# fakufaku/diffusion-separation

Hardware: AMD Instinct MI355X
Metric: separated utterances/sec (4 s, 8 kHz, 2-spk, N=30 PC steps) (higher is better)
Workload: dtype f16; 1 GPU; configs[1]: 2-spk N=30 PC sampler (+1 ald2 corrector step), batch=16 x 4.0 s @ 8 kHz per GPU and step, NCSN++ nf=64 random-init, 60 NFE/step; 4 consecutive steps (batches) in flight per GPU; batch_per_gpu=16, samples=32000, N=30, corrector_steps=1, nf=64, graph=True, batches_in_flight=4

## Files before the change

### diffusion-separation_amd/csrc/conv3x3_rw.hip

```cpp
#include <stdlib.h>

#ifdef RW_TIMING
#define HALO_TIMING rw
#endif
#include "conv3x3_halo.h"

namespace {

constexpr int KC = 64;
constexpr int NKB = KC / 16;
constexpr int KSC = 9 * NKB;
static_assert(KC * 2 + 16 == AROW && KC / 8 == PPL, "a pixel's chunk is one 128-byte line");

struct RwK {
  const bf16_t* x; long x_bs; int ldx; int C1;
  const bf16_t* x2; long x2_bs; int ldx2;
  const bf16_t* w; int w_chunked;
  const bf16_t* wfrag; const bf16_t* swfrag;
  const float* gn_scale; const float* gn_shift;
  const long long* gn_acc1; const long long* gn_acc2; const float* gn_gamma; const float* gn_beta;
  int gn_groups; float gn_inv_count; float gn_eps;
  const float* bias; const float* bias_b; int bias_b_ld;
  const bf16_t* res; long res_bs; int ldr;
  float out_scale;
  bf16_t* y; long y_bs; int ldy;
  long long* stats;
  const bf16_t* sx; long sx_bs; int ldsx; int sC1;
  const bf16_t* sx2; long sx2_bs; int ldsx2;
  const bf16_t* sw; int sw_chunked; int sw_shift; int sCin;
  int H, W, G, tiles_x, tiles_per_img;
  int dbg;
};

#ifndef RW_NWL2
#define RW_NWL2 8
#endif
constexpr int rw_lds_ksteps(int nch, int rpw, int nsk, int ncg) { return ncg == 4 ? nch * KSC - 64 + nsk * NKB : (nch == 2 ? RW_NWL2 : 0); }

template <int NCH, int RPW, int NSK, int NCG>
struct RwGeom {
  static constexpr int CO = 32 * NCG, PGN = 4 / NCG;
  static constexpr int TH = PGN * RPW, HH_ = TH + 2, HP = HH_ * HW_;
  static constexpr int NI = TH * TW * PPL / NT, NBP = HP - TH * TW, NB = (NBP * PPL + NT - 1) / NT;
  static constexpr int NL = NI + NB;
  static_assert(NT / PPL == TW && TH * TW * PPL % NT == 0, "one staging pass = one tile row");
  static constexpr int LDS_A = NL * (NT / PPL) * AROW;
  static constexpr int CIN = NCH * KC, SCIN = NSK * KC;
  static constexpr int LDS_TAB = (2 * CIN + CO) * 4;
  static constexpr int LDS_DESC = NB * NT * 4;
  static_assert((NI + NB) * (NT / PPL) >= HP + NB * (NT / PPL) - NBP, "dummy pixels of the last border pass fit the slot");
  static constexpr int NPH = NCH + NSK;
  static constexpr int NKS = NCH * KSC + NSK * NKB;
  static constexpr int NWL = rw_lds_ksteps(NCH, RPW, NSK, NCG), NWR = NKS - NWL;
  static constexpr int LDS_WL = NWL * NCG * 64 * 16;
  static constexpr int WL_STEP = NCG * 64 * 16;
  static constexpr int OFF_TAB = 2 * LDS_A, OFF_WL = OFF_TAB + ((LDS_TAB + 15) & ~15), OFF_DESC = OFF_WL + LDS_WL;
  static constexpr int LDS_TOTAL = OFF_DESC + LDS_DESC;
  static constexpr int chunk_of(int P) { return P < NSK ? NCH + P : P - NSK; }
  static_assert(LDS_TOTAL <= 160 * 1024, "LDS budget of one CU");
  static_assert(NT * 36 * 4 <= LDS_TOTAL, "the statistics reduce reuses the block's LDS");
};

template <int NCH, int RPW, int NSK, int MODE, int NCG>
__global__ __launch_bounds__(NT, 1) void conv3x3_rw_kernel(RwK p) {
  using G = RwGeom<NCH, RPW, NSK, NCG>;
  constexpr int CO = G::CO, PGN = G::PGN;
  constexpr int TH = G::TH, HP = G::HP, LDS_A = G::LDS_A, NL = G::NL, NPH = G::NPH, NKS = G::NKS, CIN = G::CIN, NWR = G::NWR;
  extern __shared__ __attribute__((aligned(16))) char smem[];
  char* sA = smem;
  float* sTab = reinterpret_cast<float*>(smem + G::OFF_TAB);
  int* sDesc = reinterpret_cast<int*>(smem + G::OFF_DESC);
  const int tid = threadIdx.x;
  const int lane = tid & 63, wave = __builtin_amdgcn_readfirstlane(tid >> 6);
  const int l32 = lane & 31, h = lane >> 5;
  const int cg = wave % NCG, pg = wave / NCG;
  const int b = blockIdx.x / p.G, part = blockIdx.x % p.G;
  const int t0 = (int)((long)part * p.tiles_per_img / p.G);
  const int nt = (int)((long)(part + 1) * p.tiles_per_img / p.G) - t0;
  RT_DECL

  static_assert(CIN <= NT && CO <= NT, "one table entry per thread");
  constexpr int CPG_MAX = 8;
  long long t_s[CPG_MAX], t_q[CPG_MAX];
  float t_gam = 1.f, t_bet = 0.f, t_sc = 1.f, t_sh = 0.f, t_bias = 0.f;
#pragma unroll
  for (int j = 0; j < CPG_MAX; ++j) { t_s[j] = 0; t_q[j] = 0; }
  if (tid < CIN) {
    const int c = tid;
    if (p.gn_acc1) {
      const int C1 = p.C1, C2 = CIN - C1;
      const int cpg = CIN / p.gn_groups, g0 = (c / cpg) * cpg;
#pragma unroll
      for (int j = 0; j < CPG_MAX; ++j) {
        if (j < cpg) {
          const int cc = g0 + j;
          const long long* src = cc < C1 ? p.gn_acc1 + ((long)b * C1 + cc) * 2 : p.gn_acc2 + ((long)b * C2 + (cc - C1)) * 2;
          t_s[j] = src[0];
          t_q[j] = src[1];
        }
      }
      t_gam = p.gn_gamma ? p.gn_gamma[c] : 1.f;
      t_bet = p.gn_beta ? p.gn_beta[c] : 0.f;
    } else if (p.gn_scale) {
      t_sc = p.gn_scale[(long)b * CIN + c];
      t_sh = p.gn_shift[(long)b * CIN + c];
    }
  }
  if (tid < CO) t_bias = (p.bias ? p.bias[tid] : 0.f) + (p.bias_b ? p.bias_b[(long)b * p.bias_b_ld + tid] : 0.f);
  auto build_tables = [&]() __attribute__((always_inline)) {
    if (tid < CIN) {
      float sc = t_sc, sh = t_sh;
      if (p.gn_acc1) {
        long long t_ssum = 0, t_ssq = 0;
#pragma unroll
        for (int j = 0; j < CPG_MAX; ++j) { t_ssum += t_s[j]; t_ssq += t_q[j]; }
        ds_gn_affine_from_acc(t_ssum, t_ssq, p.gn_inv_count, p.gn_eps, t_gam, t_bet, sc, sh);
      }
      sTab[tid] = sc;
      sTab[CIN + tid] = sh;
    }
    if (tid < CO) sTab[2 * CIN + tid] = t_bias * p.out_scale;
  };
  const int slot = tid & (PPL - 1);
  constexpr int NI = G::NI, NB = G::NB, NBP = G::NBP;
  const int ixp = tid / PPL;
  unsigned fl = 0;
  int dstb[NB];
#pragma unroll
  for (int kb = 0; kb < NB; ++kb) {
    const int bi = ixp + (NT / PPL) * kb;
    int hy, hx;
    if (bi < HW_) { hy = 0; hx = bi; }
    else if (bi < 2 * HW_) { hy = G::HH_ - 1; hx = bi - HW_; }
    else if (bi < 2 * HW_ + TH) { hy = 1 + bi - 2 * HW_; hx = 0; }
    else { hy = 1 + bi - 2 * HW_ - TH; hx = HW_ - 1; }
    const bool in = bi < NBP;
    const unsigned flg = in ? (hy == 0 ? 1u : 0u) | (hy == G::HH_ - 1 ? 2u : 0u) | (hx == 0 ? 4u : 0u) | (hx == HW_ - 1 ? 8u : 0u) : 16u;
    sDesc[kb * NT + tid] = in ? (hy - 1) * p.W + (hx - 1) : 0;
    dstb[kb] = (in ? hy * HW_ + hx : HP + (bi - NBP)) * AROW + slot * 16;
    fl |= flg << (5 * kb);
  }
  const int ldi0 = (HW_ + 1 + ixp) * AROW + slot * 16;

  RT_MARK(6)
  const int M = p.H * p.W;
  const __amdgpu_buffer_rsrc_t rx1 = rsrc(p.x + (long)b * p.x_bs, (unsigned)M * p.ldx * 2u);
  const __amdgpu_buffer_rsrc_t rx2 = p.x2 ? rsrc(p.x2 + (long)b * p.x2_bs, (unsigned)M * p.ldx2 * 2u) : rx1;
  const __amdgpu_buffer_rsrc_t rs1 = NSK ? rsrc(p.sx + (long)b * p.sx_bs, (unsigned)M * p.ldsx * 2u) : rx1;
  const __amdgpu_buffer_rsrc_t rs2 = (NSK && p.sx2) ? rsrc(p.sx2 + (long)b * p.sx2_bs, (unsigned)M * p.ldsx2 * 2u) : rs1;
  const __amdgpu_buffer_rsrc_t ry = rsrc(p.y + (long)b * p.y_bs, (unsigned)M * p.ldy * 2u);

  u32x4_t wf[NWR > 0 ? NWR : 1];
  char* sWl = smem + G::OFF_WL + (cg * 64 + lane) * 16;
  auto put_w = [&](int ks, const u32x4_t& v) __attribute__((always_inline)) {
    if (ks < NWR) wf[ks] = v;
    else if (pg == 0) *reinterpret_cast<u32x4_t*>(sWl + (ks - NWR) * G::WL_STEP) = v;
  };
  auto load_weights = [&]() __attribute__((always_inline)) {
    const bool wfm = p.wfrag != nullptr, sfm = NSK && p.swfrag != nullptr;
    const __amdgpu_buffer_rsrc_t rw = rsrc(wfm ? p.wfrag : p.w, 9u * CO * CIN * 2u);
    const __amdgpu_buffer_rsrc_t rsw = (NSK && p.sw) ? rsrc(sfm ? p.swfrag : p.sw, (unsigned)CO * G::SCIN * 2u) : rsrc(p.w, 0u);
    const unsigned vfrag = (unsigned)((cg * 64 + lane) * 16);
    const int co = cg * 32 + l32;
    const bool wc = p.w_chunked != 0;
    const unsigned vlane = wfm ? vfrag : (wc ? (unsigned)((co * 32 + h * 8) * 2) : (unsigned)((co * 9 * CIN + h * 8) * 2));
    const bool sc_ = NSK && p.sw_chunked != 0;
    const int kcs = sc_ ? p.sw_chunked : 16;
    const unsigned vl2 = sfm ? vfrag : (sc_ ? (unsigned)((co * kcs + h * 8) * 2) : (unsigned)((co * G::SCIN + h * 8) * 2));
    auto load_one = [&](int ks) __attribute__((always_inline)) {
      if (ks < NCH * KSC) {
        const int c = ks / KSC, tap = (ks % KSC) / NKB, kb = ks % NKB;
        const int chb = c * KC + kb * 16;
        const unsigned so = wfm ? (unsigned)(ks * NCG * 1024)
                                : (wc ? (unsigned)((((chb >> 5) * 9 + tap) * CO * 32 + (chb & 31)) * 2) : (unsigned)((tap * CIN + chb) * 2));
        put_w(ks, ld16v(rw, vlane, so));
      } else {
        const int chb = (ks - NCH * KSC) * 16;
        const unsigned so = sfm ? (unsigned)((ks - NCH * KSC) * NCG * 1024)
                                : (sc_ ? (unsigned)((((chb >> p.sw_shift) * CO) * kcs + (chb & (kcs - 1))) * 2) : (unsigned)(chb * 2));
        u32x4_t f = ld16v(rsw, vl2, so);
        if (!p.sw) {
          const int d = co - (chb + 8 * h);
#pragma unroll
          for (int e = 0; e < 4; ++e) f[e] = d == 2 * e ? DS_H_ONE : (d == 2 * e + 1 ? DS_H_ONE << 16 : 0u);
        }
        put_w(ks, f);
      }
    };
#pragma unroll
    for (int ks = NWR; ks < NKS; ++ks) load_one(ks);
#pragma unroll
    for (int ks = 0; ks < NWR; ++ks) load_one(ks);
  };

  u32x4_t pa[NL];
  struct TileG { int pix0; unsigned edge; };
  auto geom_at = [&](int ty, int tx, bool valid) {
    TileG g;
    const int y0 = ty * TH, x0 = tx * TW;
    g.edge = (y0 == 0 ? 1u : 0u) | (y0 + TH == p.H ? 2u : 0u) | (x0 == 0 ? 4u : 0u) | (x0 + TW == p.W ? 8u : 0u);
    g.pix0 = valid ? y0 * p.W + x0 : 0x3fffff;
    return g;
  };
  auto tile_geom = [&](int i) {
    const int t = t0 + i;
    const int ty = t / p.tiles_x;
    return geom_at(ty, t - ty * p.tiles_x, i < nt);
  };
  auto piece_ok = [&](auto P_, const TileG& g, int k) __attribute__((always_inline)) {
    constexpr int P = decltype(P_)::value;
    const unsigned em = (P < NCH ? (g.edge | 16u) : 31u) << (5 * (k - NI));
    return (fl & em) == 0u;
  };
  auto issue_one = [&](auto P_, const TileG& g, int k, int rel) __attribute__((always_inline)) {
    constexpr int P = decltype(P_)::value;
    constexpr bool CONV = P < NCH;
    constexpr int CB = (CONV ? P : P - NCH) * KC;
    const int c1 = CONV ? p.C1 : p.sC1;
    const bool second = CB >= c1;
    const unsigned ld2 = (unsigned)(CONV ? (second ? p.ldx2 : p.ldx) : (second ? p.ldsx2 : p.ldsx)) * 2u;
    const unsigned co2 = (unsigned)((second ? CB - c1 : CB) * 2) + (unsigned)slot * 16u;
    const __amdgpu_buffer_rsrc_t r = CONV ? (second ? rx2 : rx1) : (second ? rs2 : rs1);
    if constexpr (!CONV) {
      if (k >= NI) return;
    }
    if (k < NI) {
      const unsigned off = __umul24((unsigned)(g.pix0 + k * p.W + ixp), ld2) + co2;
      pa[k] = ld16v(r, off, 0);
      return;
    }
    const unsigned off = __umul24((unsigned)(rel + g.pix0), ld2) + co2;
#ifdef RW_TIMING
    pa[k] = ld16v(r, (piece_ok(P_, g, k) && !(p.dbg & 2)) ? off : OOB, 0);
#else
    pa[k] = ld16v(r, piece_ok(P_, g, k) ? off : OOB, 0);
#endif
  };
  constexpr bool FOLD = MODE == 2 && NSK == 0;
#if defined(DS_HALF_F16) && !defined(RW_ACT_F32)
  constexpr bool ACT_PK = true;
#else
  constexpr bool ACT_PK = false;
#endif
  constexpr int PIPE_LAG = 2;
  float gsc[ACT_PK ? 1 : 8], gsh[ACT_PK ? 1 : 8];
  unsigned psc[ACT_PK ? 4 : 1], psh[ACT_PK ? 4 : 1];
  auto act_tab = [&](int c) __attribute__((always_inline)) {
    if constexpr (MODE != 0) {
      const float4* ts = reinterpret_cast<const float4*>(sTab + c * KC + slot * 8);
      const float4* th = reinterpret_cast<const float4*>(sTab + CIN + c * KC + slot * 8);
      const float4 s0 = ts[0], s1 = ts[1], h0 = th[0], h1 = th[1];
      float a[8] = {s0.x, s0.y, s0.z, s0.w, s1.x, s1.y, s1.z, s1.w}, b_[8] = {h0.x, h0.y, h0.z, h0.w, h1.x, h1.y, h1.z, h1.w};
      if constexpr (FOLD) {
#pragma unroll
        for (int j = 0; j < 8; ++j) { a[j] *= -1.4426950408889634f; b_[j] *= -1.4426950408889634f; }
      }
      if constexpr (ACT_PK) {
#pragma unroll
        for (int d = 0; d < 4; ++d) { psc[d] = pack_h2(a[2 * d], a[2 * d + 1]); psh[d] = pack_h2(b_[2 * d], b_[2 * d + 1]); }
      } else {
#pragma unroll
        for (int j = 0; j < 8; ++j) { gsc[j] = a[j]; gsh[j] = b_[j]; }
      }
    }
  };
  u32x4_t so;
  float uz[3][2], ut[3][2];
  unsigned uzp[3], utp[3], uxp[3], udp[3], urp[3];
  auto unit_s01 = [&](auto P1_, int u0, int u1) __attribute__((always_inline)) {
    constexpr int P1 = decltype(P1_)::value;
    if constexpr (P1 < NCH && MODE != 0) {
      const int q0 = u0 >= 0 ? u0 % 3 : 0, q1 = u1 >= 0 ? u1 % 3 : 0;
      if constexpr (ACT_PK) {
        unsigned z = 0, x = 0, e = 0, dd = 0, r = 0;
        if (u0 >= 0) {
          asm("v_pk_fma_f16 %0, %1, %2, %3" : "=v"(z) : "v"(pa[u0 >> 2][u0 & 3]), "v"(psc[u0 & 3]), "v"(psh[u0 & 3]));
          x = z;
          if constexpr (MODE == 2 && !FOLD) asm("v_pk_mul_f16 %0, %1, %2" : "=v"(x) : "v"(z), "s"(0xbdc5bdc5u));
        }
        if constexpr (MODE == 2) {
          if (u1 >= 0) asm("v_pk_add_f16 %0, %1, %2" : "=v"(dd) : "v"(utp[q1]), "s"(0x3c003c00u));
          if (u0 >= 0) asm("v_exp_f16 %0, %1" : "=v"(e) : "v"(x));
          if (u1 >= 0) asm("v_rcp_f16 %0, %1" : "=v"(r) : "v"(dd));
          if (u0 >= 0) asm("v_exp_f16_sdwa %0, %1 dst_sel:WORD_1 dst_unused:UNUSED_PRESERVE src0_sel:WORD_1" : "+v"(e) : "v"(x));
          if (u1 >= 0) asm("v_rcp_f16_sdwa %0, %1 dst_sel:WORD_1 dst_unused:UNUSED_PRESERVE src0_sel:WORD_1" : "+v"(r) : "v"(dd));
          if (u1 >= 0) urp[q1] = r;
          if (u0 >= 0) utp[q0] = e;
        }
        if (u0 >= 0) uzp[q0] = z;
      } else {
        if (u1 >= 0 && MODE == 2) {
          ut[q1][0] = __builtin_amdgcn_rcpf(1.0f + ut[q1][0]);
          ut[q1][1] = __builtin_amdgcn_rcpf(1.0f + ut[q1][1]);
        }
        if (u0 >= 0) {
          const unsigned w = pa[u0 >> 2][u0 & 3];
          const int d = u0 & 3;
          const float lo = h_lo(w), hi = h_hi(w);
          const float z0 = fmaf(lo, gsc[2 * d], gsh[2 * d]), z1 = fmaf(hi, gsc[2 * d + 1], gsh[2 * d + 1]);
          uz[q0][0] = z0; uz[q0][1] = z1;
          if (MODE == 2) {
            ut[q0][0] = __builtin_amdgcn_exp2f(FOLD ? z0 : z0 * -1.4426950408889634f);
            ut[q0][1] = __builtin_amdgcn_exp2f(FOLD ? z1 : z1 * -1.4426950408889634f);
          }
        }
      }
    }
  };
  auto unit_s2x = [&](auto P1_, auto P2_, auto FIN_, const TileG& g1, const TileG& g2, int sl, int u, int rel) __attribute__((always_inline)) {
    constexpr int P1 = decltype(P1_)::value;
    constexpr bool FIN_ONLY = decltype(FIN_)::value;
    const int k = u >> 2, d = u & 3, q = u % 3;
    if constexpr (!FIN_ONLY) {
    if constexpr (P1 < NCH && MODE != 0) {
      if constexpr (ACT_PK) {
        unsigned v = uzp[q];
        if constexpr (MODE == 2) asm volatile("v_pk_mul_f16 %0, %1, %2" : "=v"(v) : "v"(uzp[q]), "v"(urp[q]));
        so[d] = v;
      } else {
        float z0 = uz[q][0], z1 = uz[q][1];
        if (MODE == 2) { z0 *= ut[q][0]; z1 *= ut[q][1]; }
        so[d] = pack_h2(z0, z1);
      }
    } else {
      so[d] = pa[k][d];
    }
    }
    if (d == 3) {
      if (P1 < NCH && MODE != 0 && k >= NI) {
        const bool ok = piece_ok(P1_, g1, k);
        so.x = ok ? so.x : 0u;
        so.y = ok ? so.y : 0u;
        so.z = ok ? so.z : 0u;
        so.w = ok ? so.w : 0u;
      }
#ifdef RW_ABL_NOLDSW
      asm volatile("" :: "v"(so));
#else
      if (P1 < NCH || k < NI)
        *reinterpret_cast<u32x4_t*>(sA + sl * LDS_A + (k < NI ? ldi0 + k * HW_ * AROW : dstb[k < NI ? 0 : k - NI])) = so;
#endif
#ifdef RW_ABL_NOLOAD
      pa[k][0] += rel;
#else
      issue_one(P2_, g2, k, rel);
#endif
    }
  };
  auto unit_s2 = [&](auto P1_, auto P2_, const TileG& g1, const TileG& g2, int sl, int u, int rel) __attribute__((always_inline)) {
    unit_s2x(P1_, P2_, std::false_type{}, g1, g2, sl, u, rel);
  };
  auto unit_fin = [&](auto P1_, auto P2_, const TileG& g1, const TileG& g2, int sl, int u, int rel) __attribute__((always_inline)) {
    unit_s2x(P1_, P2_, std::true_type{}, g1, g2, sl, u, rel);
  };
  auto unit = [&](auto P1_, auto P2_, const TileG& g1, const TileG& g2, int sl, int u, int rel) __attribute__((always_inline)) {
    unit_s01(P1_, u, -1);
    unit_s01(P1_, -1, u);
    unit_s2(P1_, P2_, g1, g2, sl, u, rel);
  };

  f32x16 acc[RPW];
#pragma unroll
  for (int r = 0; r < RPW; ++r)
#pragma unroll
    for (int e = 0; e < 16; ++e) acc[r][e] = 0.f;
  float ssum[16], ssq[16];
#pragma unroll
  for (int j = 0; j < 16; ++j) { ssum[j] = 0.f; ssq[j] = 0.f; }
  const bool has_stats = p.stats != nullptr;
  const float osc = FOLD ? p.out_scale * -0.6931471805599453f : p.out_scale;
  const int fbase = (pg * RPW * HW_ + l32) * AROW + h * 16;

  auto swap_halves = [&](u32x4_t& v) __attribute__((always_inline)) {
    auto r0 = __builtin_amdgcn_permlane32_swap(v.x, v.z, false, false);
    auto r1 = __builtin_amdgcn_permlane32_swap(v.y, v.w, false, false);
    v.x = r0[0]; v.z = r0[1]; v.y = r1[0]; v.w = r1[1];
  };
  u32x4_t ov0;
  const int srow = lane >> 4;
  const unsigned spiece = (unsigned)(cg * 64 + (srow & 1) * 32 + (srow >> 1) * 16);
  auto epi_unit = [&](const TileG& g, int r, int j, const float4& t0, const float4& t1) __attribute__((always_inline)) {
    float v[8];
    v[0] = fmaf(acc[r][8 * j + 0], osc, t0.x); v[1] = fmaf(acc[r][8 * j + 1], osc, t0.y);
    v[2] = fmaf(acc[r][8 * j + 2], osc, t0.z); v[3] = fmaf(acc[r][8 * j + 3], osc, t0.w);
    v[4] = fmaf(acc[r][8 * j + 4], osc, t1.x); v[5] = fmaf(acc[r][8 * j + 5], osc, t1.y);
    v[6] = fmaf(acc[r][8 * j + 6], osc, t1.z); v[7] = fmaf(acc[r][8 * j + 7], osc, t1.w);
#ifndef RW_ABL_NOSTATS
#pragma unroll
    for (int e = 0; e < 8; ++e) {
      ssum[8 * j + e] += v[e];
      ssq[8 * j + e] = fmaf(v[e], v[e], ssq[8 * j + e]);
    }
#endif
    u32x4_t ov = {pack_h2(v[0], v[1]), pack_h2(v[2], v[3]), pack_h2(v[4], v[5]), pack_h2(v[6], v[7])};
    swap_halves(ov);
    if (j == 0) {
      ov0 = ov;
    } else {
      u32x4_t a = ov0, b2 = ov;
#pragma unroll
      for (int d = 0; d < 4; ++d) {
        auto q = __builtin_amdgcn_permlane16_swap(a[d], b2[d], false, false);
        a[d] = q[0]; b2[d] = q[1];
      }
      const int pix = g.pix0 + (pg * RPW + r) * p.W + (lane & 15);
      const unsigned o = __umul24((unsigned)pix, (unsigned)p.ldy * 2u) + spiece;
#ifdef RW_TIMING
      const unsigned o1 = (p.dbg & 1) ? OOB : o, o2 = (p.dbg & 1) ? OOB : o + 16u * (unsigned)p.ldy * 2u;
#else
      const unsigned o1 = o, o2 = o + 16u * (unsigned)p.ldy * 2u;
#endif
#ifdef RW_ABL_NOSTORE
      asm volatile("" :: "v"(a), "v"(b2), "v"(o1), "v"(o2));
#else
      __builtin_amdgcn_raw_buffer_store_b128(a, ry, o1, 0, 0);
      __builtin_amdgcn_raw_buffer_store_b128(b2, ry, o2, 0, 0);
#endif
    }
  };
  constexpr bool REL_REGS = NWR * 4 <= 176 || NCG == 4;
  constexpr bool BIAS_REGS = true;
  float4 breg[2][2];
  int relreg[G::NB];
  auto epi_bias = [&](int j, float4& t0, float4& t1) __attribute__((always_inline)) {
    if constexpr (BIAS_REGS) {
      t0 = breg[j][0];
      t1 = breg[j][1];
    } else {
      t0 = *reinterpret_cast<const float4*>(sTab + 2 * CIN + cg * 32 + 8 * (2 * j) + 4 * h);
      t1 = *reinterpret_cast<const float4*>(sTab + 2 * CIN + cg * 32 + 8 * (2 * j + 1) + 4 * h);
    }
  };

  constexpr int RH = RPW / 2;
#ifndef RW_W_E
#define RW_W_E 2
#define RW_W_N 5
#endif
  constexpr int W_E = RW_W_E, W_N = RW_W_N;
  float et[2][2] = {{0.f, 0.f}, {0.f, 0.f}};
  u32x4_t osa = {0, 0, 0, 0}, osb = {0, 0, 0, 0};
  auto half = [&](auto P_, auto HF_, auto EPI_, int slot_r, const TileG& ge, const TileG& g1, const TileG& g2) __attribute__((always_inline)) {
    constexpr int P = decltype(P_)::value, HF = decltype(HF_)::value;
    constexpr bool EPI = decltype(EPI_)::value;
    constexpr int C = G::chunk_of(P);
    constexpr bool CONV = C < NCH;
    constexpr int NK = CONV ? KSC : NKB;
    constexpr int W0 = CONV ? C * KSC : NCH * KSC + (C - NCH) * NKB;
    constexpr int C1 = G::chunk_of((P + 1) % NPH), C2 = G::chunk_of((P + 2) % NPH);
    constexpr int NU = NL * 4;
    constexpr bool ACT1 = C1 < NCH && MODE != 0;
    constexpr int LAG = ACT1 ? PIPE_LAG : 0, NUV = NU + LAG, NLU = 2 * NUV;
    constexpr int NGH = NK * RH;
    constexpr int w0 = (P == 0) ? W_E : W_N, w1 = (P == NPH - 1) ? W_E : W_N, CAP = NGH * (w0 + w1);
    auto lub = [](int GP) constexpr { return NLU * (GP <= NGH ? GP * w0 : NGH * w0 + (GP - NGH) * w1) / CAP; };
    constexpr int NLE = RH * 22;
    constexpr int R0 = HF * RH, ER0 = HF ? 0 : RH;
    const char* fb = sA + slot_r * LDS_A + fbase + R0 * HW_ * AROW;
#ifndef RW_BUILTIN_MFMA
    if constexpr (EPI) {
#pragma unroll
      for (int r = 0; r < RH; ++r) asm volatile("s_nop 11" : "+v"(acc[ER0 + r]));
    }
#endif
    if constexpr (HF == 0 && C1 < NCH) act_tab(C1);
    constexpr int SUB = CONV ? 3 : 1, RFN = CONV ? RH + 2 : RH, NG = NK / SUB;
    static_assert(SUB * RH >= RFN, "the next group's fragments are read in the MFMA slots of the current one");
    auto ldg = [&](int g, int j) __attribute__((always_inline)) {
      const int dx = CONV ? g / NKB : 1, kb = g % NKB, row = CONV ? j : j + 1;
      return *reinterpret_cast<const u32x4_t*>(fb + (row * HW_ + dx) * AROW + kb * 32);
    };
    u32x4_t rf[2][RFN];
#pragma unroll
    for (int j = 0; j < RFN; ++j) rf[0][j] = ldg(0, j);
    auto widx = [](int ks) {
      if (!CONV) return ks;
      const int g = ks / 3, dy = ks % 3, dx = g / NKB, kb = g % NKB;
      return (dy * 3 + dx) * NKB + kb;
    };
#define RW_FRAG(ks, r) rf[((ks) / SUB) & 1][(r) + (CONV ? (ks) % SUB : 0)]
#define RW_FRAG_LAST(ks) rf[((ks) / SUB) & 1][RFN - 1]
    u32x4_t wl = {0, 0, 0, 0}, wln = {0, 0, 0, 0};
    if constexpr (W0 + widx(0) >= NWR) wl = *reinterpret_cast<const u32x4_t*>(sWl + (W0 + widx(0) - NWR) * G::WL_STEP);
    int rels[2][NL];
    auto fetch_rels = [&](int ks, int par) __attribute__((always_inline)) {
      const int gp0 = HF * NGH + ks * RH;
#pragma unroll
      for (int L = lub(gp0); L < lub(gp0 + RH); ++L) {
        const int u = (L >> 1) - LAG;
        if ((L & 1) && u >= 0 && u < NU && (u & 3) == 3 && (u >> 2) >= NI)
          rels[par][u >> 2] = REL_REGS ? relreg[(u >> 2) - NI] : sDesc[((u >> 2) - NI) * NT + tid];
      }
    };
    fetch_rels(0, 0);

    auto unit_lump = [&](int L, int par) __attribute__((always_inline)) {
      const int v = L >> 1;
      const int u0 = v < NU ? v : -1, u1 = LAG ? ((v >= 1 && v - 1 < NU) ? v - 1 : -1) : v, u2 = v - LAG;
      const bool s2 = u2 >= 0 && u2 < NU;
      if ((L & 1) == 0) {
        if constexpr (ACT1 && ACT_PK) {
          if (u0 >= 0) {
            asm volatile("v_pk_fma_f16 %0, %1, %2, %3" : "=v"(uzp[u0 % 3]) : "v"(pa[u0 >> 2][u0 & 3]), "v"(psc[u0 & 3]), "v"(psh[u0 & 3]));
            if constexpr (MODE == 2 && !FOLD) asm volatile("v_pk_mul_f16 %0, %1, %2" : "=v"(uxp[u0 % 3]) : "v"(uzp[u0 % 3]), "s"(0xbdc5bdc5u));
          }
          if constexpr (MODE == 2) {
            if (u1 >= 0) asm volatile("v_pk_add_f16 %0, %1, %2" : "=v"(udp[u1 % 3]) : "v"(utp[u1 % 3]), "s"(0x3c003c00u));
            if (s2) asm volatile("v_pk_mul_f16 %0, %1, %2" : "=v"(so[u2 & 3]) : "v"(uzp[u2 % 3]), "v"(urp[u2 % 3]));
            if (u0 >= 0) asm volatile("v_exp_f16 %0, %1" : "=v"(utp[u0 % 3]) : "v"(FOLD ? uzp[u0 % 3] : uxp[u0 % 3]));
            if (u1 >= 0) asm volatile("v_rcp_f16 %0, %1" : "=v"(urp[u1 % 3]) : "v"(udp[u1 % 3]));
          } else {
            if (s2) so[u2 & 3] = uzp[u2 % 3];
          }
        } else if constexpr (ACT1) {
          if (u0 >= 0) unit_s01(std::integral_constant<int, C1>{}, u0, -1);
        }
      } else {
        if constexpr (ACT1 && ACT_PK) {
          if constexpr (MODE == 2) {
            if (u0 >= 0) asm volatile("v_exp_f16_sdwa %0, %1 dst_sel:WORD_1 dst_unused:UNUSED_PRESERVE src0_sel:WORD_1" : "+v"(utp[u0 % 3]) : "v"(FOLD ? uzp[u0 % 3] : uxp[u0 % 3]));
            if (u1 >= 0) asm volatile("v_rcp_f16_sdwa %0, %1 dst_sel:WORD_1 dst_unused:UNUSED_PRESERVE src0_sel:WORD_1" : "+v"(urp[u1 % 3]) : "v"(udp[u1 % 3]));
          }
        } else if constexpr (ACT1) {
          if (u1 >= 0) unit_s01(std::integral_constant<int, C1>{}, -1, u1);
        }
#ifndef RW_ABL_NOSTAGE
        if (s2) {
          const int rel = ((u2 & 3) == 3 && (u2 >> 2) >= NI) ? rels[par][u2 >> 2] : 0;
          if constexpr (ACT1 && ACT_PK) unit_fin(std::integral_constant<int, C1>{}, std::integral_constant<int, C2>{}, g1, g2, slot_r ^ 1, u2, rel);
          else unit_s2(std::integral_constant<int, C1>{}, std::integral_constant<int, C2>{}, g1, g2, slot_r ^ 1, u2, rel);
        }
#endif
      }
    };
    auto epi_lump = [&](int LE) __attribute__((always_inline)) {
      const int rr = ER0 + LE / 22, x = LE % 22;
      if (x < 20) {
        const int j = x / 10, y = x % 10;
        const bool isA = y == 0 || y == 1 || y == 3 || y == 5 || y == 7;
        const int pr = y == 0 ? 0 : (y == 1 ? 1 : (y == 2 ? 0 : (y == 3 ? 2 : (y == 4 ? 1 : (y == 5 ? 3 : (y == 6 ? 2 : (y == 7 ? 4 : 3)))))));
        if (y == 9) {
          if (j == 0) {
            asm volatile("v_permlane32_swap_b32 %0, %1" : "+v"(osa[0]), "+v"(osa[2]));
            asm volatile("v_permlane32_swap_b32 %0, %1" : "+v"(osa[1]), "+v"(osa[3]));
          } else {
            asm volatile("v_permlane32_swap_b32 %0, %1" : "+v"(osb[0]), "+v"(osb[2]));
            asm volatile("v_permlane32_swap_b32 %0, %1" : "+v"(osb[1]), "+v"(osb[3]));
          }
        } else if (isA) {
          if (pr < 4) {
            const int e0 = 8 * j + 2 * pr;
            const float b0 = pr == 0 ? breg[j][0].x : (pr == 1 ? breg[j][0].z : (pr == 2 ? breg[j][1].x : breg[j][1].z));
            const float b1 = pr == 0 ? breg[j][0].y : (pr == 1 ? breg[j][0].w : (pr == 2 ? breg[j][1].y : breg[j][1].w));
            asm volatile("v_fma_f32 %0, %1, %2, %3" : "=v"(et[pr & 1][0]) : "v"(acc[rr][e0]), "s"(osc), "v"(b0));
            asm volatile("v_fma_f32 %0, %1, %2, %3" : "=v"(et[pr & 1][1]) : "v"(acc[rr][e0 + 1]), "s"(osc), "v"(b1));
          }
          if (pr >= 1) {
            const int q = pr - 1;
            if (j == 0) asm volatile(DS_CVT_PK_H_ASM " %0, %1, %2" : "=v"(osa[q]) : "v"(et[q & 1][0]), "v"(et[q & 1][1]));
            else asm volatile(DS_CVT_PK_H_ASM " %0, %1, %2" : "=v"(osb[q]) : "v"(et[q & 1][0]), "v"(et[q & 1][1]));
          }
        } else {
#ifndef RW_ABL_NOSTATS
          const int e0 = 8 * j + 2 * pr;
          asm volatile("v_add_f32 %0, %0, %1" : "+v"(ssum[e0]) : "v"(et[pr & 1][0]));
          asm volatile("v_add_f32 %0, %0, %1" : "+v"(ssum[e0 + 1]) : "v"(et[pr & 1][1]));
          asm volatile("v_fma_f32 %0, %1, %1, %0" : "+v"(ssq[e0]) : "v"(et[pr & 1][0]));
          asm volatile("v_fma_f32 %0, %1, %1, %0" : "+v"(ssq[e0 + 1]) : "v"(et[pr & 1][1]));
#endif
        }
      } else if (x == 20) {
#pragma unroll
        for (int d = 0; d < 4; ++d) asm volatile("v_permlane16_swap_b32 %0, %1" : "+v"(osa[d]), "+v"(osb[d]));
      } else {
        const int pix = ge.pix0 + (pg * RPW + rr) * p.W + (lane & 15);
        const unsigned o = __umul24((unsigned)pix, (unsigned)p.ldy * 2u) + spiece;
#ifdef RW_TIMING
        const unsigned o1 = (p.dbg & 1) ? OOB : o, o2 = (p.dbg & 1) ? OOB : o + 16u * (unsigned)p.ldy * 2u;
#else
        const unsigned o1 = o, o2 = o + 16u * (unsigned)p.ldy * 2u;
#endif
#ifdef RW_ABL_NOSTORE
        asm volatile("" :: "v"(osa), "v"(osb), "v"(o1), "v"(o2));
#else
        __builtin_amdgcn_raw_buffer_store_b128(osa, ry, o1, 0, 0);
        __builtin_amdgcn_raw_buffer_store_b128(osb, ry, o2, 0, 0);
#endif
      }
    };

#pragma unroll
    for (int ks = 0; ks < NK; ++ks) {
      if (ks + 1 < NK) fetch_rels(ks + 1, (ks + 1) & 1);
      const int wi = W0 + widx(ks), win = W0 + widx(ks + 1 < NK ? ks + 1 : ks);
      if (win >= NWR && ks + 1 < NK) wln = *reinterpret_cast<const u32x4_t*>(sWl + (win - NWR) * G::WL_STEP);
      const u32x4_t wk = wi < NWR ? wf[wi < NWR ? wi : 0] : wl;
#define RW_DEP , "v"(RW_FRAG_LAST(ks))
#pragma unroll
      for (int r = 0; r < RH; ++r) {
        if (wi < NWR) {
          if (P == 0 && ks == 0) asm volatile(DS_MFMA_H32_ASM " %0, %1, %2, 0" : "=v"(acc[R0 + r]) : "a"(wk), "v"(RW_FRAG(ks, r)) RW_DEP);
          else asm volatile(DS_MFMA_H32_ASM " %0, %1, %2, %0" : "+v"(acc[R0 + r]) : "a"(wk), "v"(RW_FRAG(ks, r)) RW_DEP);
        } else {
          if (P == 0 && ks == 0) asm volatile(DS_MFMA_H32_ASM " %0, %1, %2, 0" : "=v"(acc[R0 + r]) : "v"(wk), "v"(RW_FRAG(ks, r)) RW_DEP);
          else asm volatile(DS_MFMA_H32_ASM " %0, %1, %2, %0" : "+v"(acc[R0 + r]) : "v"(wk), "v"(RW_FRAG(ks, r)) RW_DEP);
        }
        {
          const int g = ks / SUB, q = (ks % SUB) * RH + r;
          if (q < RFN && g + 1 < NG) rf[(g + 1) & 1][q] = ldg(g + 1, q);
        }
        const int gh = ks * RH + r, gp = HF * NGH + gh;
#pragma unroll
        for (int L = lub(gp); L < lub(gp + 1); ++L) unit_lump(L, ks & 1);
#ifndef RW_ABL_NOEPI
        if constexpr (EPI) {
#pragma unroll
          for (int LE = gh * NLE / NGH; LE < (gh + 1) * NLE / NGH; ++LE) epi_lump(LE);
        }
#endif
      }
      wl = wln;
      __builtin_amdgcn_sched_barrier(0);
    }
  };

  TileG gc = tile_geom(0);
  constexpr int CH0 = G::chunk_of(0), CH1 = G::chunk_of(1 % NPH);
  const TileG g1st = NPH > 1 ? gc : tile_geom(1);
  {
#pragma unroll
    for (int k = 0; k < NL; ++k) issue_one(std::integral_constant<int, CH0>{}, gc, k, k < NI ? 0 : sDesc[(k < NI ? 0 : k - NI) * NT + tid]);
    load_weights();
    build_tables();
    sync_lds();
    RT_MARK(7)
    if constexpr (REL_REGS) {
#pragma unroll
      for (int k = 0; k < NB; ++k) relreg[k] = sDesc[k * NT + tid];
    }
    if constexpr (BIAS_REGS) {
#pragma unroll
      for (int j = 0; j < 2; ++j) {
        breg[j][0] = *reinterpret_cast<const float4*>(sTab + 2 * CIN + cg * 32 + 8 * (2 * j) + 4 * h);
        breg[j][1] = *reinterpret_cast<const float4*>(sTab + 2 * CIN + cg * 32 + 8 * (2 * j + 1) + 4 * h);
      }
    }
    act_tab(CH0);
#pragma unroll
    for (int u = 0; u < NL * 4; ++u)
      unit(std::integral_constant<int, CH0>{}, std::integral_constant<int, CH1>{}, gc, g1st, 0, u,
           (u >> 2) < NI ? 0 : sDesc[((u >> 2) < NI ? 0 : (u >> 2) - NI) * NT + tid]);
  }
  RT_MARK(0)
  TileG gp = tile_geom(nt);
  int ph = 0;
  TileG gnc = tile_geom(1);
  int ty2 = (t0 + 2) / p.tiles_x, tx2 = (t0 + 2) - ty2 * p.tiles_x;
  for (int i = 0; i < nt; ++i) {
    const TileG gn = gnc, gnn = geom_at(ty2, tx2, i + 2 < nt);
    auto run = [&](auto self, auto P_) __attribute__((always_inline)) {
      constexpr int P = decltype(P_)::value;
      sync_lds();
      RT_MARK(1)
      const int slot_r = ph & 1;
      half(P_, std::integral_constant<int, 0>{}, std::integral_constant<bool, P == 0>{}, slot_r, gp, ((P + 1) / NPH == 0 ? gc : gn), ((P + 2) / NPH == 0 ? gc : ((P + 2) / NPH == 1 ? gn : gnn)));
      if constexpr (P == 0) {
        if (i == 0) {
#pragma unroll
          for (int j = 0; j < 16; ++j) { ssum[j] = 0.f; ssq[j] = 0.f; }
        }
      }
      half(P_, std::integral_constant<int, 1>{}, std::integral_constant<bool, P == NPH - 1>{}, slot_r, gc, ((P + 1) / NPH == 0 ? gc : gn), ((P + 2) / NPH == 0 ? gc : ((P + 2) / NPH == 1 ? gn : gnn)));
      ++ph;
      RT_MARK(G::chunk_of(P) < NCH ? 2 : 3)
      if constexpr (P + 1 < NPH) self(self, std::integral_constant<int, P + 1>{});
    };
    run(run, std::integral_constant<int, 0>{});
    gp = gc;
    gc = gn;
    gnc = gnn;
    if (++tx2 == p.tiles_x) { tx2 = 0; ++ty2; }
  }
#ifndef RW_BUILTIN_MFMA
#pragma unroll
  for (int r = 0; r < RH; ++r) asm volatile("s_nop 11" : "+v"(acc[RH + r]));
#endif
#pragma unroll
  for (int e = 0; e < RH * 2; ++e) {
    float4 t0, t1;
    epi_bias(e & 1, t0, t1);
    epi_unit(gp, RH + (e >> 1), e & 1, t0, t1);
  }
  RT_MARK(4)
  if (has_stats) {
    __syncthreads();
    float* red = reinterpret_cast<float*>(smem);
    constexpr int RED_ROW = 36;
#pragma unroll
    for (int q = 0; q < 4; ++q) {
      *reinterpret_cast<float4*>(red + tid * RED_ROW + 4 * q) = make_float4(ssum[4 * q], ssum[4 * q + 1], ssum[4 * q + 2], ssum[4 * q + 3]);
      *reinterpret_cast<float4*>(red + tid * RED_ROW + 16 + 4 * q) = make_float4(ssq[4 * q], ssq[4 * q + 1], ssq[4 * q + 2], ssq[4 * q + 3]);
    }
    __syncthreads();
    if (tid < 2 * CO) {
      const int co = tid >> 1, st = tid & 1;
      const int wcg = co >> 5, c32 = co & 31, q = c32 >> 3, hh = (c32 >> 2) & 1, i = c32 & 3;
      double a = 0.0;
      for (int wpg = 0; wpg < PGN; ++wpg)
        for (int l = 0; l < 32; ++l) {
          const int t = (wpg * NCG + wcg) * 64 + hh * 32 + l;
          a += (double)red[t * RED_ROW + st * 16 + 4 * q + i];
        }
      ds_stat_flush(p.stats + ((long)b * CO + co) * 2, st, a);
    }
  }
  RT_MARK(5)
  RT_FLUSH
}

int rw_blocks_per_image(const ConvArgs& a, int tiles) {
  int g = ds_num_cus() / a.B;
#ifdef RW_TIMING
  if (getenv("DIFFSEP_RW_G")) g = atoi(getenv("DIFFSEP_RW_G"));
#endif
  if ((a.opts & DS_OPT_RW_HALF) && g >= 2 && tiles / g <= 4) g /= 2;
  if ((a.opts & DS_OPT_RW_QUARTER) && g >= 4 && tiles / g <= 4) g /= 4;
  if ((a.opts & DS_OPT_RW_BIG_HALF) && g >= 2 && tiles / g > 4) g /= 2;
  if (g < 1) g = 1;
  if (g > tiles) g = tiles;
  return g;
}

template <int NCH, int RPW, int NSK, int MODE, int NCG>
int rw_launch(const RwK& k0, const ConvArgs& a, hipStream_t st) {
  using G = RwGeom<NCH, RPW, NSK, NCG>;
  RwK k = k0;
  const int tiles = (a.H / G::TH) * (a.W / TW);
  k.G = rw_blocks_per_image(a, tiles);
  k.tiles_x = a.W / TW;
  k.tiles_per_img = tiles;
  auto kern = conv3x3_rw_kernel<NCH, RPW, NSK, MODE, NCG>;
  DS_FUNC_LDS_ONCE(kern, G::LDS_TOTAL);
  hipLaunchKernelGGL(kern, dim3(a.B * k.G), dim3(NT), G::LDS_TOTAL, st, k);
  DS_LAUNCH_CHECK();
  {
    static char name[64] = {0};
    if (!name[0]) snprintf(name, sizeof(name), "conv3x3_rw_kernel<%d,%d,%d,%d,%d>", NCH, RPW, NSK, MODE, NCG);
    ds_set_last_conv_kernel(name);
  }
  return 0;
}

}

bool ds_conv_rw_supported(const ConvArgs& a) {
  const int CO = a.Cout;
  if (!(a.dtype == DS_BF16 && a.taps == 9 && ((CO == 64 && (a.Cin == 64 || a.Cin == 128)) || (CO == 128 && a.Cin == 128)) &&
        a.w_bs == 0 && (a.w_chunked == 0 || a.w_chunked == 32) && a.bias_mode == 0 && !a.div_b && a.W % TW == 0 && a.H % 8 == 0 &&
        a.H >= 32 && a.W >= 32 && a.ldy >= CO && a.ldy % 8 == 0 && (!a.res || (a.ldr >= CO && a.ldr % 8 == 0))))
    return false;
  if (a.x2 ? !(a.C1 % KC == 0 && a.C1 > 0 && a.C1 < a.Cin && a.ldx % 8 == 0 && a.ldx2 % 8 == 0) : a.ldx % 8 != 0) return false;
  const bool gn = a.gn_scale || a.gn_acc1;
  if (gn && !a.gn_act) return false;
  if (a.gn_acc1 && !(a.gn_groups > 0 && a.Cin % a.gn_groups == 0 && a.Cin / a.gn_groups <= 8 && (!a.x2 || a.gn_acc2))) return false;
  if (a.sx) {
    if (!(a.sw && !a.res && (a.sCin == 64 || a.sCin == 128 || (a.sCin == 192 && CO == 64 && a.Cin == 64)) && a.ldsx % 8 == 0 &&
          (!a.sx2 || (a.sC1 % KC == 0 && a.sC1 > 0 && a.sC1 < a.sCin && a.ldsx2 % 8 == 0)) &&
          (a.sw_chunked == 0 || ((a.sw_chunked & (a.sw_chunked - 1)) == 0 && a.sw_chunked >= 16))))
      return false;
    if (a.Cin == 128 && CO == 64) return false;
  }
  if (a.res && a.Cin == 128 && CO == 64) return false;
  if (CO == 128 && (a.sx || a.res) && !gn) return false;
  return true;
}

int ds_launch_conv_rw(const ConvArgs& a, hipStream_t st) {
  RwK k;
  k.x = reinterpret_cast<const bf16_t*>(a.x); k.x_bs = a.x_bs; k.ldx = a.ldx; k.C1 = a.x2 ? a.C1 : a.Cin;
  k.x2 = reinterpret_cast<const bf16_t*>(a.x2); k.x2_bs = a.x2_bs; k.ldx2 = a.x2 ? a.ldx2 : a.ldx;
  k.w = reinterpret_cast<const bf16_t*>(a.w); k.w_chunked = a.w_chunked;
  k.wfrag = reinterpret_cast<const bf16_t*>(a.w_frag);
  k.swfrag = (a.sx && a.sw) ? reinterpret_cast<const bf16_t*>(a.sw_frag) : nullptr;
  k.gn_scale = a.gn_scale; k.gn_shift = a.gn_shift;
  k.gn_acc1 = a.gn_acc1; k.gn_acc2 = a.gn_acc2; k.gn_gamma = a.gn_gamma; k.gn_beta = a.gn_beta;
  k.gn_groups = a.gn_groups; k.gn_inv_count = a.gn_inv_count; k.gn_eps = a.gn_eps;
  k.bias = a.bias; k.bias_b = a.bias_b; k.bias_b_ld = a.bias_b_ld;
  k.res = reinterpret_cast<const bf16_t*>(a.res); k.res_bs = a.res_bs; k.ldr = a.ldr;
  k.out_scale = a.out_scale;
  k.y = reinterpret_cast<bf16_t*>(a.y); k.y_bs = a.y_bs; k.ldy = a.ldy;
  k.stats = a.stats_acc;
  k.sx = reinterpret_cast<const bf16_t*>(a.sx); k.sx_bs = a.sx_bs; k.ldsx = a.ldsx; k.sC1 = a.sx2 ? a.sC1 : a.sCin;
  k.sx2 = reinterpret_cast<const bf16_t*>(a.sx2); k.sx2_bs = a.sx2_bs; k.ldsx2 = a.sx2 ? a.ldsx2 : a.ldsx;
  k.sw = reinterpret_cast<const bf16_t*>(a.sw); k.sw_chunked = a.sw_chunked; k.sw_shift = a.sw_chunked ? __builtin_ctz(a.sw_chunked) : 0;
  k.sCin = a.sCin;
  k.H = a.H; k.W = a.W; k.G = 0; k.tiles_x = 0; k.tiles_per_img = 0;
#ifdef RW_TIMING
  k.dbg = getenv("DIFFSEP_RW_DBG") ? atoi(getenv("DIFFSEP_RW_DBG")) : 0;
#else
  k.dbg = 0;
#endif
  if (a.res) {
    k.sx = reinterpret_cast<const bf16_t*>(a.res); k.sx_bs = a.res_bs; k.ldsx = a.ldr; k.sC1 = a.Cout;
    k.sx2 = nullptr; k.sx2_bs = 0; k.ldsx2 = a.ldr; k.sw = nullptr; k.sw_chunked = 0; k.sw_shift = 0; k.sCin = a.Cout;
  }
  const int mode = ((a.gn_scale || a.gn_acc1) && a.gn_act) ? 2 : 0;
  const int nsk = a.sx ? a.sCin / KC : (a.res ? a.Cout / KC : 0);
  if (a.Cout == 128) {
    if (mode == 0) return rw_launch<2, 4, 0, 0, 4>(k, a, st);
    if (nsk == 0) return rw_launch<2, 4, 0, 2, 4>(k, a, st);
    if (nsk == 1) return rw_launch<2, 4, 1, 2, 4>(k, a, st);
    return rw_launch<2, 4, 2, 2, 4>(k, a, st);
  }
#define RW_GO(NCH_, NSK_) return mode == 2 ? rw_launch<NCH_, 4, NSK_, 2, 2>(k, a, st) : rw_launch<NCH_, 4, NSK_, 0, 2>(k, a, st)
  if (a.Cin == 128) RW_GO(2, 0);
  if (nsk == 0) RW_GO(1, 0);
  if (nsk == 1) RW_GO(1, 1);
  if (nsk == 2) RW_GO(1, 2);
  RW_GO(1, 3);
#undef RW_GO
}
```

Baseline: 75.27 utterances/s.

## Stream register weight fragments into the first tile's MFMA units instead of loading upfront

Weight loading in the prologue is split. LDS-resident fragments are loaded first and stored after the table build. Only the first few register fragments are loaded before the sync, and the rest are interleaved with the first tile's compute units so their latency overlaps with MFMA work. Identity fragments for the skip path are now synthesized separately rather than patched after load. The stats reduction switches to sync_lds and an unrolled batched LDS read before the double accumulation. This adds register pressure and scheduling barriers, which may hurt occupancy.

```diff
diff --git a/diffusion-separation_amd/csrc/conv3x3_rw.hip b/diffusion-separation_amd/csrc/conv3x3_rw.hip
--- a/diffusion-separation_amd/csrc/conv3x3_rw.hip
+++ b/diffusion-separation_amd/csrc/conv3x3_rw.hip
@@ -82,7 +82,7 @@
   static_assert(CIN <= NT && CO <= NT, "one table entry per thread");
   constexpr int CPG_MAX = 8;
   long long t_s[CPG_MAX], t_q[CPG_MAX];
-  float t_gam = 1.f, t_bet = 0.f, t_sc = 1.f, t_sh = 0.f, t_bias = 0.f;
+  float t_gam = 1.f, t_bet = 0.f, t_sc = 1.f, t_sh = 0.f, t_bias = 0.f, t_bias_b = 0.f;
 #pragma unroll
   for (int j = 0; j < CPG_MAX; ++j) { t_s[j] = 0; t_q[j] = 0; }
   if (tid < CIN) {
@@ -106,7 +106,10 @@
       t_sh = p.gn_shift[(long)b * CIN + c];
     }
   }
-  if (tid < CO) t_bias = (p.bias ? p.bias[tid] : 0.f) + (p.bias_b ? p.bias_b[(long)b * p.bias_b_ld + tid] : 0.f);
+  if (tid < CO) {
+    if (p.bias) t_bias = p.bias[tid];
+    if (p.bias_b) t_bias_b = p.bias_b[(long)b * p.bias_b_ld + tid];
+  }
   auto build_tables = [&]() __attribute__((always_inline)) {
     if (tid < CIN) {
       float sc = t_sc, sh = t_sh;
@@ -119,7 +122,7 @@
       sTab[tid] = sc;
       sTab[CIN + tid] = sh;
     }
-    if (tid < CO) sTab[2 * CIN + tid] = t_bias * p.out_scale;
+    if (tid < CO) sTab[2 * CIN + tid] = (t_bias + t_bias_b) * p.out_scale;
   };
   const int slot = tid & (PPL - 1);
   constexpr int NI = G::NI, NB = G::NB, NBP = G::NBP;
@@ -152,45 +155,66 @@
 
   u32x4_t wf[NWR > 0 ? NWR : 1];
   char* sWl = smem + G::OFF_WL + (cg * 64 + lane) * 16;
-  auto put_w = [&](int ks, const u32x4_t& v) __attribute__((always_inline)) {
-    if (ks < NWR) wf[ks] = v;
-    else if (pg == 0) *reinterpret_cast<u32x4_t*>(sWl + (ks - NWR) * G::WL_STEP) = v;
-  };
-  auto load_weights = [&]() __attribute__((always_inline)) {
-    const bool wfm = p.wfrag != nullptr, sfm = NSK && p.swfrag != nullptr;
-    const __amdgpu_buffer_rsrc_t rw = rsrc(wfm ? p.wfrag : p.w, 9u * CO * CIN * 2u);
-    const __amdgpu_buffer_rsrc_t rsw = (NSK && p.sw) ? rsrc(sfm ? p.swfrag : p.sw, (unsigned)CO * G::SCIN * 2u) : rsrc(p.w, 0u);
-    const unsigned vfrag = (unsigned)((cg * 64 + lane) * 16);
-    const int co = cg * 32 + l32;
-    const bool wc = p.w_chunked != 0;
-    const unsigned vlane = wfm ? vfrag : (wc ? (unsigned)((co * 32 + h * 8) * 2) : (unsigned)((co * 9 * CIN + h * 8) * 2));
-    const bool sc_ = NSK && p.sw_chunked != 0;
-    const int kcs = sc_ ? p.sw_chunked : 16;
-    const unsigned vl2 = sfm ? vfrag : (sc_ ? (unsigned)((co * kcs + h * 8) * 2) : (unsigned)((co * G::SCIN + h * 8) * 2));
-    auto load_one = [&](int ks) __attribute__((always_inline)) {
-      if (ks < NCH * KSC) {
-        const int c = ks / KSC, tap = (ks % KSC) / NKB, kb = ks % NKB;
-        const int chb = c * KC + kb * 16;
-        const unsigned so = wfm ? (unsigned)(ks * NCG * 1024)
-                                : (wc ? (unsigned)((((chb >> 5) * 9 + tap) * CO * 32 + (chb & 31)) * 2) : (unsigned)((tap * CIN + chb) * 2));
-        put_w(ks, ld16v(rw, vlane, so));
-      } else {
-        const int chb = (ks - NCH * KSC) * 16;
-        const unsigned so = sfm ? (unsigned)((ks - NCH * KSC) * NCG * 1024)
-                                : (sc_ ? (unsigned)((((chb >> p.sw_shift) * CO) * kcs + (chb & (kcs - 1))) * 2) : (unsigned)(chb * 2));
-        u32x4_t f = ld16v(rsw, vl2, so);
-        if (!p.sw) {
-          const int d = co - (chb + 8 * h);
-#pragma unroll
-          for (int e = 0; e < 4; ++e) f[e] = d == 2 * e ? DS_H_ONE : (d == 2 * e + 1 ? DS_H_ONE << 16 : 0u);
-        }
-        put_w(ks, f);
-      }
-    };
-#pragma unroll
-    for (int ks = NWR; ks < NKS; ++ks) load_one(ks);
-#pragma unroll
-    for (int ks = 0; ks < NWR; ++ks) load_one(ks);
+  u32x4_t wl_in[G::NWL > 0 ? G::NWL : 1];
+  const bool wfm = p.wfrag != nullptr, sfm = NSK && p.swfrag != nullptr;
+  const __amdgpu_buffer_rsrc_t rw = rsrc(wfm ? p.wfrag : p.w, 9u * CO * CIN * 2u);
+  const __amdgpu_buffer_rsrc_t rsw = (NSK && p.sw) ? rsrc(sfm ? p.swfrag : p.sw, (unsigned)CO * G::SCIN * 2u) : rsrc(p.w, 0u);
+  const unsigned vfrag = (unsigned)((cg * 64 + lane) * 16);
+  const int co = cg * 32 + l32;
+  const bool wc = p.w_chunked != 0;
+  const unsigned vlane = wfm ? vfrag : (wc ? (unsigned)((co * 32 + h * 8) * 2) : (unsigned)((co * 9 * CIN + h * 8) * 2));
+  const bool sc_ = NSK && p.sw_chunked != 0;
+  const int kcs = sc_ ? p.sw_chunked : 16;
+  const unsigned vl2 = sfm ? vfrag : (sc_ ? (unsigned)((co * kcs + h * 8) * 2) : (unsigned)((co * G::SCIN + h * 8) * 2));
+  auto load_one = [&](int ks) __attribute__((always_inline)) -> u32x4_t {
+    if (ks < NCH * KSC) {
+      const int c = ks / KSC, tap = (ks % KSC) / NKB, kb = ks % NKB;
+      const int chb = c * KC + kb * 16;
+      const unsigned so = wfm ? (unsigned)(ks * NCG * 1024)
+                              : (wc ? (unsigned)((((chb >> 5) * 9 + tap) * CO * 32 + (chb & 31)) * 2) : (unsigned)((tap * CIN + chb) * 2));
+      return ld16v(rw, vlane, so);
+    } else {
+      const int chb = (ks - NCH * KSC) * 16;
+      const unsigned so = sfm ? (unsigned)((ks - NCH * KSC) * NCG * 1024)
+                              : (sc_ ? (unsigned)((((chb >> p.sw_shift) * CO) * kcs + (chb & (kcs - 1))) * 2) : (unsigned)(chb * 2));
+      return ld16v(rsw, vl2, so);
+    }
+  };
+  auto ident_frag = [&](int ks) __attribute__((always_inline)) -> u32x4_t {
+    const int chb = (ks - NCH * KSC) * 16;
+    const int d = co - (chb + 8 * h);
+    u32x4_t f;
+#pragma unroll
+    for (int e = 0; e < 4; ++e) f[e] = d == 2 * e ? DS_H_ONE : (d == 2 * e + 1 ? DS_H_ONE << 16 : 0u);
+    return f;
+  };
+  constexpr int NSR = NWR > NCH * KSC ? NWR - NCH * KSC : 0;
+  auto reg_frag_at = [](int i) constexpr { return i < NSR ? NCH * KSC + i : i - NSR; };
+  auto store_lds_weights = [&]() __attribute__((always_inline)) {
+    if constexpr (G::NWL > 0) {
+      if (pg == 0) {
+#pragma unroll
+        for (int j = 0; j < G::NWL; ++j) {
+          u32x4_t v = wl_in[j];
+          if (NSK > 0 && NWR + j >= NCH * KSC && !p.sw) v = ident_frag(NWR + j);
+          *reinterpret_cast<u32x4_t*>(sWl + j * G::WL_STEP) = v;
+        }
+      }
+    }
+  };
+  auto load_lds_frags = [&]() __attribute__((always_inline)) {
+    if constexpr (G::NWL > 0) {
+      if (pg == 0) {
+#pragma unroll
+        for (int ks = NWR; ks < NKS; ++ks) wl_in[ks - NWR] = load_one(ks);
+      }
+      __builtin_amdgcn_sched_barrier(0);
+    }
+  };
+  auto load_reg_frags = [&](int lo, int hi) __attribute__((always_inline)) {
+#pragma unroll
+    for (int i = lo; i < hi; ++i) wf[reg_frag_at(i)] = load_one(reg_frag_at(i));
+    __builtin_amdgcn_sched_barrier(0);
   };
 
   u32x4_t pa[NL];
@@ -630,8 +654,11 @@
   {
 #pragma unroll
     for (int k = 0; k < NL; ++k) issue_one(std::integral_constant<int, CH0>{}, gc, k, k < NI ? 0 : sDesc[(k < NI ? 0 : k - NI) * NT + tid]);
-    load_weights();
+    constexpr int NU0 = NL * 4, W_HEAD = NWR < 8 ? NWR : 8;
+    load_lds_frags();
+    load_reg_frags(0, W_HEAD);
     build_tables();
+    store_lds_weights();
     sync_lds();
     RT_MARK(7)
     if constexpr (REL_REGS) {
@@ -647,9 +674,17 @@
     }
     act_tab(CH0);
 #pragma unroll
-    for (int u = 0; u < NL * 4; ++u)
+    for (int u = 0; u < NU0; ++u) {
       unit(std::integral_constant<int, CH0>{}, std::integral_constant<int, CH1>{}, gc, g1st, 0, u,
            (u >> 2) < NI ? 0 : sDesc[((u >> 2) < NI ? 0 : (u >> 2) - NI) * NT + tid]);
+      load_reg_frags(W_HEAD + (NWR - W_HEAD) * u / NU0, W_HEAD + (NWR - W_HEAD) * (u + 1) / NU0);
+    }
+    if constexpr (NSR > 0) {
+      if (!p.sw) {
+#pragma unroll
+        for (int ks = NCH * KSC; ks < NWR; ++ks) wf[ks] = ident_frag(ks);
+      }
+    }
   }
   RT_MARK(0)
   TileG gp = tile_geom(nt);
@@ -693,7 +728,7 @@
   }
   RT_MARK(4)
   if (has_stats) {
-    __syncthreads();
+    sync_lds();
     float* red = reinterpret_cast<float*>(smem);
     constexpr int RED_ROW = 36;
 #pragma unroll
@@ -701,16 +736,21 @@
       *reinterpret_cast<float4*>(red + tid * RED_ROW + 4 * q) = make_float4(ssum[4 * q], ssum[4 * q + 1], ssum[4 * q + 2], ssum[4 * q + 3]);
       *reinterpret_cast<float4*>(red + tid * RED_ROW + 16 + 4 * q) = make_float4(ssq[4 * q], ssq[4 * q + 1], ssq[4 * q + 2], ssq[4 * q + 3]);
     }
-    __syncthreads();
+    sync_lds();
     if (tid < 2 * CO) {
       const int co = tid >> 1, st = tid & 1;
       const int wcg = co >> 5, c32 = co & 31, q = c32 >> 3, hh = (c32 >> 2) & 1, i = c32 & 3;
-      double a = 0.0;
+      float rv[PGN * 32];
+#pragma unroll
       for (int wpg = 0; wpg < PGN; ++wpg)
+#pragma unroll
         for (int l = 0; l < 32; ++l) {
           const int t = (wpg * NCG + wcg) * 64 + hh * 32 + l;
-          a += (double)red[t * RED_ROW + st * 16 + 4 * q + i];
-        }
+          rv[wpg * 32 + l] = red[t * RED_ROW + st * 16 + 4 * q + i];
+        }
+      double a = 0.0;
+#pragma unroll
+      for (int j = 0; j < PGN * 32; ++j) a += (double)rv[j];
       ds_stat_flush(p.stats + ((long)b * CO + co) * 2, st, a);
     }
   }
```

Result: no change. 75.49 utterances/s (median of 6 runs) (+0.3%).
